# stateless-consensus/phant

Measured on NVIDIA H100. Metric: mpt_proofs_verified_per_sec, higher is better.
Workload: dtype u64

## Files before the change

phant_b200/csrc/keccak_f1600.cuh:

```cuda
#pragma once
#include <stdint.h>

namespace phant {

__constant__ uint64_t KECCAK_RC[24] = {
    0x0000000000000001ull, 0x0000000000008082ull, 0x800000000000808aull, 0x8000000080008000ull,
    0x000000000000808bull, 0x0000000080000001ull, 0x8000000080008081ull, 0x8000000000008009ull,
    0x000000000000008aull, 0x0000000000000088ull, 0x0000000080008009ull, 0x000000008000000aull,
    0x000000008000808bull, 0x800000000000008bull, 0x8000000000008089ull, 0x8000000000008003ull,
    0x8000000000008002ull, 0x8000000000000080ull, 0x000000000000800aull, 0x800000008000000aull,
    0x8000000080008081ull, 0x8000000000008080ull, 0x0000000080000001ull, 0x8000000080008008ull};

constexpr int KECCAK_RATE = 136;
constexpr int KECCAK_RATE_WORDS = 17;

template <int N>
__device__ __forceinline__ uint64_t rol64(uint64_t x)
{
    if constexpr (N == 0) return x;
    const uint32_t lo = (uint32_t)x, hi = (uint32_t)(x >> 32);
    uint32_t rlo, rhi;
    if constexpr (N == 32) {
        rlo = hi; rhi = lo;
    } else if constexpr (N < 32) {
        rlo = __funnelshift_l(hi, lo, N);
        rhi = __funnelshift_l(lo, hi, N);
    } else {
        rlo = __funnelshift_l(lo, hi, N - 32);
        rhi = __funnelshift_l(hi, lo, N - 32);
    }
    return ((uint64_t)rhi << 32) | rlo;
}

#define PHANT_RHOPI(I, J, R) b[J] = rol64<R>(a[I] ^ c[((I) % 5 + 4) % 5] ^ r1[((I) % 5 + 1) % 5]);

__device__ __forceinline__ void keccak_round(uint64_t (&a)[25], uint64_t rc)
{
    uint64_t c[5], r1[5], b[25];
#pragma unroll
    for (int x = 0; x < 5; ++x) c[x] = a[x] ^ a[x + 5] ^ a[x + 10] ^ a[x + 15] ^ a[x + 20];
#pragma unroll
    for (int x = 0; x < 5; ++x) r1[x] = rol64<1>(c[x]);
    PHANT_RHOPI(0, 0, 0)    PHANT_RHOPI(1, 10, 1)   PHANT_RHOPI(2, 20, 62)  PHANT_RHOPI(3, 5, 28)   PHANT_RHOPI(4, 15, 27)
    PHANT_RHOPI(5, 16, 36)  PHANT_RHOPI(6, 1, 44)   PHANT_RHOPI(7, 11, 6)   PHANT_RHOPI(8, 21, 55)  PHANT_RHOPI(9, 6, 20)
    PHANT_RHOPI(10, 7, 3)   PHANT_RHOPI(11, 17, 10) PHANT_RHOPI(12, 2, 43)  PHANT_RHOPI(13, 12, 25) PHANT_RHOPI(14, 22, 39)
    PHANT_RHOPI(15, 23, 41) PHANT_RHOPI(16, 8, 45)  PHANT_RHOPI(17, 18, 15) PHANT_RHOPI(18, 3, 21)  PHANT_RHOPI(19, 13, 8)
    PHANT_RHOPI(20, 14, 18) PHANT_RHOPI(21, 24, 2)  PHANT_RHOPI(22, 9, 61)  PHANT_RHOPI(23, 19, 56) PHANT_RHOPI(24, 4, 14)
#pragma unroll
    for (int y = 0; y < 25; y += 5) {
#pragma unroll
        for (int x = 0; x < 5; ++x) a[y + x] = b[y + x] ^ (~b[y + (x + 1) % 5] & b[y + (x + 2) % 5]);
    }
    a[0] ^= rc;
}

__device__ __forceinline__ void keccak_last_round_digest(uint64_t (&a)[25], uint64_t rc)
{
    uint64_t c[5], r1[5], b[5];
#pragma unroll
    for (int x = 0; x < 5; ++x) c[x] = a[x] ^ a[x + 5] ^ a[x + 10] ^ a[x + 15] ^ a[x + 20];
#pragma unroll
    for (int x = 0; x < 5; ++x) r1[x] = rol64<1>(c[x]);
    PHANT_RHOPI(0, 0, 0) PHANT_RHOPI(6, 1, 44) PHANT_RHOPI(12, 2, 43) PHANT_RHOPI(18, 3, 21) PHANT_RHOPI(24, 4, 14)
#pragma unroll
    for (int x = 0; x < 4; ++x) a[x] = b[x] ^ (~b[(x + 1) % 5] & b[(x + 2) % 5]);
    a[0] ^= rc;
}
#undef PHANT_RHOPI

template <int UNROLL = 2, bool DIGEST_ONLY = false>
__device__ __forceinline__ void keccak_f1600(uint64_t (&a)[25])
{
    constexpr int LOOPED = DIGEST_ONLY ? 24 - UNROLL : 24;
#pragma unroll 1
    for (int r = 0; r < LOOPED; r += UNROLL) {
#pragma unroll
        for (int k = 0; k < UNROLL; ++k) keccak_round(a, KECCAK_RC[r + k]);
    }
    if constexpr (DIGEST_ONLY) {
#pragma unroll
        for (int k = 0; k < UNROLL - 1; ++k) keccak_round(a, KECCAK_RC[LOOPED + k]);
        keccak_last_round_digest(a, KECCAK_RC[23]);
    }
}

struct MsgView {
    const uint64_t* w;
    uint32_t sh;
};
__device__ __forceinline__ MsgView msg_view(const void* p)
{
    const uintptr_t a = (uintptr_t)p;
    return MsgView{(const uint64_t*)(a & ~(uintptr_t)7), (uint32_t)(a & 7) * 8};
}
__device__ __forceinline__ uint64_t funnel64(uint64_t lo, uint64_t hi, uint32_t sh)
{
    return sh ? (lo >> sh) | (hi << (64 - sh)) : lo;
}

template <int UNROLL>
__device__ __forceinline__ void absorb_full(uint64_t (&st)[25], const MsgView& v, uint32_t base)
{
    uint64_t w[KECCAK_RATE_WORDS + 1];
#pragma unroll
    for (int k = 0; k < KECCAK_RATE_WORDS; ++k) w[k] = v.w[base + k];
    w[KECCAK_RATE_WORDS] = v.sh ? v.w[base + KECCAK_RATE_WORDS] : 0;
#pragma unroll
    for (int k = 0; k < KECCAK_RATE_WORDS; ++k) st[k] ^= funnel64(w[k], w[k + 1], v.sh);
    keccak_f1600<UNROLL>(st);
}

template <int UNROLL>
__device__ __forceinline__ void absorb_final(uint64_t (&st)[25], const MsgView& v, uint32_t base, uint32_t rem)
{
    const uint32_t mis = v.sh >> 3;
#pragma unroll
    for (int k = 0; k < KECCAK_RATE_WORDS; ++k) {
        const int valid = (int)rem - 8 * k;
        uint64_t word = 0;
        if (valid > 0) {
            const uint64_t lo = v.w[base + k];
            const uint64_t hi = (mis + (valid > 8 ? 8 : valid) > 8) ? v.w[base + k + 1] : 0;
            word = funnel64(lo, hi, v.sh);
            if (valid < 8) word &= (1ull << (8 * valid)) - 1;
        }
        if (valid >= 0 && valid < 8) word ^= 1ull << (8 * valid);
        st[k] ^= word;
    }
    st[KECCAK_RATE_WORDS - 1] ^= 0x8000000000000000ull;
    keccak_f1600<UNROLL, true>(st);
}

#ifndef PHANT_HOST_SMEM
__device__ __forceinline__ uint32_t lds32(uint32_t saddr)
{
    uint32_t v;
    asm volatile("ld.shared.u32 %0, [%1];" : "=r"(v) : "r"(saddr));
    return v;
}
#else
__device__ __forceinline__ uint32_t lds32(uint32_t saddr) { uint32_t v; memcpy(&v, PHANT_HOST_SMEM + saddr, 4); return v; }
#endif
template <int UNROLL, bool DIGEST_ONLY = false>
__device__ __forceinline__ void absorb_full_smem(uint64_t (&st)[25], uint32_t sa)
{
    const uint32_t a4 = sa & ~3u, sh = (sa & 3u) * 8;
    uint32_t w[2 * KECCAK_RATE_WORDS + 1];
#pragma unroll
    for (int j = 0; j < 2 * KECCAK_RATE_WORDS; ++j) w[j] = lds32(a4 + 4 * j);
    w[2 * KECCAK_RATE_WORDS] = sh ? lds32(a4 + 4 * 2 * KECCAK_RATE_WORDS) : 0;
#pragma unroll
    for (int k = 0; k < KECCAK_RATE_WORDS; ++k) {
        const uint32_t lo = __funnelshift_r(w[2 * k], w[2 * k + 1], sh);
        const uint32_t hi = __funnelshift_r(w[2 * k + 1], w[2 * k + 2], sh);
        st[k] ^= ((uint64_t)hi << 32) | lo;
    }
    keccak_f1600<UNROLL, DIGEST_ONLY>(st);
}
#ifndef PHANT_HOST_SMEM
__device__ __forceinline__ void sts32_(uint32_t saddr, uint32_t v) { asm volatile("st.shared.u32 [%0], %1;" ::"r"(saddr), "r"(v) : "memory"); }
#else
__device__ __forceinline__ void sts32_(uint32_t saddr, uint32_t v) { memcpy(PHANT_HOST_SMEM + saddr, &v, 4); }
#endif
template <int UNROLL>
__device__ __forceinline__ void absorb_final_smem_masked(uint64_t (&st)[25], uint32_t sa, uint32_t rem)
{
    const uint32_t a4 = sa & ~3u, sh = (sa & 3u) * 8;
    const uint32_t nfw = rem >> 2, tail = rem & 3u;
    const uint32_t bmask = (1u << (8 * tail)) - 1u, pad = 1u << (8 * tail);
    uint32_t prev = rem ? lds32(a4) : 0;
#pragma unroll
    for (int j = 0; j < 2 * KECCAK_RATE_WORDS; ++j) {
        uint32_t word = 0;
        if ((uint32_t)j < nfw || ((uint32_t)j == nfw && tail)) {
            const uint32_t next = lds32(a4 + 4 * (j + 1));
            word = __funnelshift_r(prev, next, sh);
            prev = next;
        }
        if ((uint32_t)j == nfw) word = (word & bmask) ^ pad;
        if (j == 2 * KECCAK_RATE_WORDS - 1) word ^= 0x80000000u;
        st[j >> 1] ^= (j & 1) ? ((uint64_t)word << 32) : (uint64_t)word;
    }
    keccak_f1600<UNROLL, true>(st);
}
template <int UNROLL>
__device__ __forceinline__ void absorb_final_smem(uint64_t (&st)[25], uint32_t sa, uint32_t rem, uint32_t room)
{
    if (room < KECCAK_RATE + 4) { absorb_final_smem_masked<UNROLL>(st, sa, rem); return; }
    const uint32_t a4 = sa & ~3u, s = sa & 3u;
    const uint32_t p0 = rem + s, p1 = KECCAK_RATE - 1 + s;
    const uint32_t q0 = p0 >> 2, b0 = p0 & 3u, q1 = p1 >> 2, b1 = p1 & 3u;
    uint32_t w0 = lds32(a4 + 4 * q0);
    w0 = (w0 & ((1u << (8 * b0)) - 1u)) | (1u << (8 * b0));
    if (q0 == q1) w0 |= 0x80u << (8 * b1);
    sts32_(a4 + 4 * q0, w0);
    for (uint32_t q = q0 + 1; q < q1; ++q) sts32_(a4 + 4 * q, 0u);
    if (q1 > q0) sts32_(a4 + 4 * q1, 0x80u << (8 * b1));
    absorb_full_smem<UNROLL, true>(st, sa);
}

template <int UNROLL = 2>
__device__ __forceinline__ void keccak256_thread(const uint8_t* p, uint64_t len, uint64_t (&digest)[4])
{
    uint64_t st[25];
#pragma unroll
    for (int i = 0; i < 25; ++i) st[i] = 0;
    const MsgView v = msg_view(p);
    uint32_t base = 0;
    while (len >= KECCAK_RATE) {
        absorb_full<UNROLL>(st, v, base);
        base += KECCAK_RATE_WORDS;
        len -= KECCAK_RATE;
    }
    absorb_final<UNROLL>(st, v, base, (uint32_t)len);
#pragma unroll
    for (int i = 0; i < 4; ++i) digest[i] = st[i];
}

}
```

phant_b200/csrc/keccak_kernels.cu:

```cuda
#include "common.cuh"
#include "keccak_f1600.cuh"
#include "node_summary.cuh"
#include "stage.cuh"

#include <stdlib.h>
#include <string.h>

namespace phant {

template <int UNROLL>
__global__ void __launch_bounds__(128)
keccak256_direct_kernel(const uint8_t* __restrict__ msgs, const uint64_t* __restrict__ off,
                        const uint32_t* __restrict__ order, uint64_t n, uint8_t* __restrict__ out,
                        uint32_t* __restrict__ summary, const uint64_t* __restrict__ len)
{
    for (uint64_t i = (uint64_t)blockIdx.x * blockDim.x + threadIdx.x; i < n; i += (uint64_t)gridDim.x * blockDim.x) {
        const uint64_t m = order ? order[i] : i;
        const uint64_t beg = off[m], end = len ? beg + len[m] : off[m + 1];
        uint64_t dg[4];
        keccak256_thread<UNROLL>(msgs + beg, end - beg, dg);
        if (summary) summary[m] = (end - beg) <= 4096 ? summarize_node(msgs + beg, (uint32_t)(end - beg)) : 0;
        uint64_t* o = reinterpret_cast<uint64_t*>(out + 32 * m);
        o[0] = dg[0]; o[1] = dg[1]; o[2] = dg[2]; o[3] = dg[3];
    }
}


template <int UNROLL, int BLOCKS, int WARPS>
__global__ void __launch_bounds__(WARPS * 32)
keccak256_staged_kernel(const uint8_t* __restrict__ msgs, const uint64_t* __restrict__ off,
                        const uint32_t* __restrict__ order, uint64_t n, uint8_t* __restrict__ out,
                        uint32_t* __restrict__ summary, const uint64_t* __restrict__ len)
{
    extern __shared__ __align__(128) uint8_t smem[];
    const uint32_t warp = threadIdx.x >> 5, lane = threadIdx.x & 31;
    const uint32_t bar = smem_u32(smem) + 8 * warp;
    constexpr int SLOT = stage_slot(BLOCKS), WINDOW = stage_window(BLOCKS);
    uint8_t* slot = smem + 128 + (warp * 32 + lane) * SLOT;
    const uint32_t slot_s = smem_u32(slot);
    if (lane == 0) mbar_init(bar, 32);
    fence_proxy_async();
    __syncthreads();
    uint32_t parity = 0;

    const uint64_t n_tiles = (n + 31) / 32;
    for (uint64_t tile = (uint64_t)blockIdx.x * WARPS + warp; tile < n_tiles; tile += (uint64_t)gridDim.x * WARPS) {
        const uint64_t idx = tile * 32 + lane;
        const bool active = idx < n;
        uint64_t m = 0, cur = 0, end = 0;
        if (active) {
            m = order ? order[idx] : idx;
            cur = off[m];
            end = len ? cur + len[m] : off[m + 1];
        }
        uint64_t st[25];
#pragma unroll
        for (int i = 0; i < 25; ++i) st[i] = 0;
        bool done = !active;
        bool first_trip = true;

        while (!__all_sync(0xffffffffu, done)) {
            const uint64_t need = done ? 0 : end - cur;
            const uint64_t a0 = cur & ~(uint64_t)15;
            uint32_t cs = 0;
            if (need) {
                const uint64_t span = ((end - a0) + 15) & ~(uint64_t)15;
                cs = span < WINDOW ? (uint32_t)span : WINDOW;
                fence_proxy_async();
                mbar_arrive_expect_tx(bar, cs);
                bulk_g2s(slot_s, msgs + a0, cs, bar);
            } else {
                mbar_arrive(bar);
            }
            mbar_wait(bar, parity);
            parity ^= 1;
            if (!done) {
                const uint32_t skew = (uint32_t)(cur - a0);
                const uint64_t in_slot = cs - skew;
                const uint64_t avail = need < in_slot ? need : in_slot;
                if (summary && first_trip)
                    summary[m] = avail == need ? summarize_node(slot + skew, (uint32_t)need) : 0;
                const uint32_t nfull = (uint32_t)(avail / KECCAK_RATE);
                uint32_t sa = slot_s + skew;
                for (uint32_t b = 0; b < nfull; ++b) {
                    absorb_full_smem<UNROLL>(st, sa);
                    sa += KECCAK_RATE;
                }
                if (avail == need) {
                    absorb_final_smem<UNROLL>(st, sa, (uint32_t)(avail - (uint64_t)nfull * KECCAK_RATE), slot_s + SLOT - sa);
                    done = true;
                } else {
                    cur += (uint64_t)nfull * KECCAK_RATE;
                }
            }
            first_trip = false;
        }
        if (active) {
            uint4* o = reinterpret_cast<uint4*>(out + 32 * m);
            o[0] = make_uint4((uint32_t)st[0], (uint32_t)(st[0] >> 32), (uint32_t)st[1], (uint32_t)(st[1] >> 32));
            o[1] = make_uint4((uint32_t)st[2], (uint32_t)(st[2] >> 32), (uint32_t)st[3], (uint32_t)(st[3] >> 32));
        }
    }
}

__device__ __forceinline__ uint64_t rolv64(uint64_t x, uint32_t n) { return n ? (x << n) | (x >> (64 - n)) : x; }

__global__ void __launch_bounds__(256)
keccak256_warp_kernel(const uint8_t* __restrict__ msgs, const uint64_t* __restrict__ off, uint64_t n,
                      uint8_t* __restrict__ out, const uint64_t* __restrict__ lens)
{
    const uint32_t lane = threadIdx.x & 31;
    const uint64_t warp_id = ((uint64_t)blockIdx.x * blockDim.x + threadIdx.x) >> 5;
    const uint64_t n_warps = ((uint64_t)gridDim.x * blockDim.x) >> 5;
    const uint32_t x = lane % 5, y = (lane % 25) / 5;
    constexpr uint32_t RHO[25] = {0, 1, 62, 28, 27, 36, 44, 6, 55, 20, 3, 10, 43, 25, 39, 41, 45, 15, 21, 8, 18, 2, 61, 56, 14};
    uint32_t rho = 0;
#pragma unroll
    for (int i = 0; i < 25; ++i) if (lane == (uint32_t)i) rho = RHO[i];
    const uint32_t pi_src = ((x + 3 * y) % 5) + 5 * x;
    const uint32_t col1 = (x + 1) % 5, col4 = (x + 4) % 5;
    const uint32_t row1 = 5 * y + (x + 1) % 5, row2 = 5 * y + (x + 2) % 5;
    const uint32_t FULL = 0xffffffffu;

    for (uint64_t m = warp_id; m < n; m += n_warps) {
        const uint64_t beg = off[m], end = lens ? beg + lens[m] : off[m + 1];
        uint64_t len = end - beg;
        const MsgView v = msg_view(msgs + beg);
        uint64_t s = 0;
        uint32_t base = 0;
        bool last = false;
        while (!last) {
            uint64_t word = 0;
            if (len >= KECCAK_RATE) {
                uint64_t lo = 0;
                if (lane <= KECCAK_RATE_WORDS && (lane < KECCAK_RATE_WORDS || v.sh)) lo = v.w[base + lane];
                const uint64_t hi = __shfl_down_sync(FULL, lo, 1);
                word = lane < KECCAK_RATE_WORDS ? funnel64(lo, hi, v.sh) : 0;
                len -= KECCAK_RATE;
                base += KECCAK_RATE_WORDS;
            } else {
                const uint32_t rem = (uint32_t)len, mis = v.sh >> 3;
                const uint32_t n_al = (mis + rem + 7) / 8;
                uint64_t lo = (rem && lane < n_al) ? v.w[base + lane] : 0;
                const uint64_t hi = __shfl_down_sync(FULL, lo, 1);
                if (lane < KECCAK_RATE_WORDS) {
                    const int valid = (int)rem - 8 * (int)lane;
                    if (valid > 0) {
                        word = funnel64(lo, hi, v.sh);
                        if (valid < 8) word &= (1ull << (8 * valid)) - 1;
                    }
                    if (valid >= 0 && valid < 8) word ^= 1ull << (8 * valid);
                    if (lane == KECCAK_RATE_WORDS - 1) word ^= 0x8000000000000000ull;
                }
                last = true;
            }
            s ^= word;
#pragma unroll 1
            for (int r = 0; r < 24; ++r) {
                uint64_t c = s;
                c ^= __shfl_sync(FULL, s, (lane + 5) % 25);
                c ^= __shfl_sync(FULL, s, (lane + 10) % 25);
                c ^= __shfl_sync(FULL, s, (lane + 15) % 25);
                c ^= __shfl_sync(FULL, s, (lane + 20) % 25);
                const uint64_t cm = __shfl_sync(FULL, c, col4), cp = __shfl_sync(FULL, c, col1);
                s ^= cm ^ rolv64(cp, 1);
                s = rolv64(s, rho);
                s = __shfl_sync(FULL, s, pi_src);
                const uint64_t b1 = __shfl_sync(FULL, s, row1), b2 = __shfl_sync(FULL, s, row2);
                s ^= ~b1 & b2;
                if (lane == 0) s ^= KECCAK_RC[r];
            }
        }
        if (lane < 4) reinterpret_cast<uint64_t*>(out + 32 * m)[lane] = s;
    }
}

constexpr int CLS_THREADS = 256, CLS_WARPS = CLS_THREADS / 32;

__device__ __forceinline__ uint32_t keccak_class_of(uint64_t len)
{
    const uint64_t nb = len / KECCAK_RATE + 1;
    return (uint32_t)(15 - (nb > 16 ? 15 : nb - 1));
}
__device__ __forceinline__ uint32_t proof_class_of(uint64_t n_nodes) { return (uint32_t)(15 - (n_nodes > 15 ? 15 : n_nodes)); }
template <bool PROOFS>
__device__ __forceinline__ uint32_t class_of(uint64_t len) { return PROOFS ? proof_class_of(len) : keccak_class_of(len); }

template <bool PROOFS>
__global__ void __launch_bounds__(CLS_THREADS)
keccak_class_kernel(const uint64_t* __restrict__ off, uint64_t n, uint64_t chunk, uint32_t* __restrict__ hist ,
                    uint32_t* __restrict__ ticket, unsigned long long* __restrict__ perms)
{
    __shared__ uint32_t h[16];
    __shared__ uint32_t cls_total[16];
    __shared__ bool last;
    if (threadIdx.x < 16) h[threadIdx.x] = 0;
    __syncthreads();
    const uint64_t lo = (uint64_t)blockIdx.x * chunk, hi = lo + chunk < n ? lo + chunk : n;
    unsigned long long local = 0;
    for (uint64_t i0 = lo; i0 < hi; i0 += CLS_THREADS) {
        const uint64_t i = i0 + threadIdx.x;
        const bool valid = i < hi;
        uint32_t c = 16;
        if (valid) {
            const uint64_t len = off[i + 1] - off[i];
            c = class_of<PROOFS>(len);
            if (!PROOFS) local += len / KECCAK_RATE + 1;
        }
        const uint32_t peers = __match_any_sync(0xffffffffu, c);
        if (valid && (threadIdx.x & 31) == (uint32_t)(__ffs(peers) - 1)) atomicAdd(&h[c], __popc(peers));
    }
    for (int o = 16; o; o >>= 1) local += __shfl_down_sync(0xffffffffu, local, o);
    if ((threadIdx.x & 31) == 0 && local) atomicAdd(perms, local);
    __syncthreads();
    if (threadIdx.x < 16) hist[16 * blockIdx.x + threadIdx.x] = h[threadIdx.x];
    __threadfence();
    __syncthreads();
    if (threadIdx.x == 0) last = atomicAdd(ticket, 1u) == gridDim.x - 1;
    __syncthreads();
    if (!last) return;
    __threadfence();
    const uint32_t nb = gridDim.x, warp = threadIdx.x >> 5, lane = threadIdx.x & 31;
    for (uint32_t c = warp; c < 16; c += CLS_WARPS) {
        uint32_t t = 0;
        for (uint32_t b = lane; b < nb; b += 32) t += __ldcg(&hist[16 * b + c]);
        for (int o = 16; o; o >>= 1) t += __shfl_down_sync(0xffffffffu, t, o);
        if (lane == 0) cls_total[c] = t;
    }
    __syncthreads();
    for (uint32_t c = warp; c < 16; c += CLS_WARPS) {
        uint32_t carry = 0;
        for (uint32_t k = 0; k < c; ++k) carry += cls_total[k];
        for (uint32_t b0 = 0; b0 < nb; b0 += 32) {
            const uint32_t b = b0 + lane;
            const uint32_t v = b < nb ? __ldcg(&hist[16 * b + c]) : 0;
            uint32_t incl = v;
            for (int o = 1; o < 32; o <<= 1) {
                const uint32_t up = __shfl_up_sync(0xffffffffu, incl, o);
                if (lane >= (uint32_t)o) incl += up;
            }
            if (b < nb) hist[16 * b + c] = carry + incl - v;
            carry += __shfl_sync(0xffffffffu, incl, 31);
// ... 154 lines not shown
```

phant_b200/csrc/verify_fused.cu:

```cuda
#include "common.cuh"
#include "stage.cuh"
#include "verify_fused.cuh"

namespace phant {

template <int UNROLL, int BLOCKS, int WARPS>
__global__ void __launch_bounds__(WARPS * 32)
verify_fused_kernel(const uint8_t* __restrict__ nodes, const uint64_t* __restrict__ node_off, const uint64_t* __restrict__ proof_first,
                    const uint32_t* __restrict__ order, uint64_t n, const uint8_t* __restrict__ keys32, const uint8_t* __restrict__ roots32,
                    uint64_t n_roots, uint8_t* __restrict__ status, uint64_t* __restrict__ val_off, uint32_t* __restrict__ val_len,
                    unsigned long long* __restrict__ perms)
{
    extern __shared__ __align__(128) uint8_t smem[];
    const uint32_t warp = threadIdx.x >> 5, lane = threadIdx.x & 31;
    const uint32_t bar = smem_u32(smem) + 8 * warp;
    constexpr int SLOT = stage_slot(BLOCKS), WINDOW = stage_window(BLOCKS);
    uint8_t* slot = smem + 128 + (warp * 32 + lane) * SLOT;
    const uint32_t slot_s = smem_u32(slot);
    if (lane == 0) mbar_init(bar, 32);
    fence_proxy_async();
    __syncthreads();
    uint32_t parity = 0;
    unsigned long long my_perms = 0;

    const uint64_t n_tiles = (n + 31) / 32;
    for (uint64_t tile = (uint64_t)blockIdx.x * WARPS + warp; tile < n_tiles; tile += (uint64_t)gridDim.x * WARPS) {
        const uint64_t idx = tile * 32 + lane;
        const bool active = idx < n;
        uint64_t p = 0;
        FusedLane L;
        L.done = true;
        if (active) {
            p = order ? order[idx] : idx;
            fused_begin(L, node_off, proof_first[p], proof_first[p + 1], keys32 + 32 * p, roots32 + (n_roots == 1 ? 0 : 32 * p));
        }
        while (!__all_sync(0xffffffffu, L.done)) {
            uint64_t a0 = 0;
            const uint32_t cs = L.done ? 0 : fused_window<WINDOW>(L, a0);
            if (cs) {
                fence_proxy_async();
                mbar_arrive_expect_tx(bar, cs);
                bulk_g2s(slot_s, nodes + a0, cs, bar);
            } else {
                mbar_arrive(bar);
            }
            mbar_wait(bar, parity);
            parity ^= 1;
            if (!L.done) fused_step<UNROLL, SLOT>(L, nodes, node_off, slot_s, slot, cs);
        }
        if (active) {
            status[p] = (uint8_t)L.status;
            if (val_off) val_off[p] = L.voff;
            if (val_len) val_len[p] = L.vlen;
            my_perms += L.perms;
        }
    }
    for (int o = 16; o; o >>= 1) my_perms += __shfl_down_sync(0xffffffffu, my_perms, o);
    if (lane == 0 && my_perms) atomicAdd(perms, my_perms);
}

cudaError_t launch_verify_fused(cudaStream_t s, int device, const uint8_t* nodes, const uint64_t* node_off, const uint64_t* proof_first,
                                const uint32_t* order, uint64_t n, const uint8_t* keys32, const uint8_t* roots32, uint64_t n_roots,
                                uint8_t* status, uint64_t* val_off, uint32_t* val_len, unsigned long long* perms)
{
    if (n == 0) return cudaSuccess;
    constexpr int BLOCKS = 4, WARPS = 12;
    constexpr int SMEM = stage_smem(BLOCKS, WARPS);
    static int ctas_cache[64] = {0};
    int& ctas_per_sm = ctas_cache[(device >= 0 && device < 64) ? device : 0];
    if (!ctas_per_sm) {
        cudaError_t e = cudaFuncSetAttribute(verify_fused_kernel<2, BLOCKS, WARPS>, cudaFuncAttributeMaxDynamicSharedMemorySize, SMEM);
        if (e != cudaSuccess) return e;
        cudaFuncSetAttribute(verify_fused_kernel<2, BLOCKS, WARPS>, cudaFuncAttributePreferredSharedMemoryCarveout, 100);
        e = cudaOccupancyMaxActiveBlocksPerMultiprocessor(&ctas_per_sm, verify_fused_kernel<2, BLOCKS, WARPS>, WARPS * 32, SMEM);
        if (e != cudaSuccess || ctas_per_sm < 1) { ctas_per_sm = 0; return e != cudaSuccess ? e : cudaErrorLaunchOutOfResources; }
    }
    const uint64_t tiles = (n + 31) / 32;
    uint64_t blocks = (tiles + WARPS - 1) / WARPS;
    const uint64_t cap = (uint64_t)keccak_num_sms(device) * ctas_per_sm;
    if (blocks > cap) blocks = cap;
    verify_fused_kernel<2, BLOCKS, WARPS><<<(unsigned)blocks, WARPS * 32, SMEM, s>>>(nodes, node_off, proof_first, order, n, keys32, roots32,
                                                                                    n_roots, status, val_off, val_len, perms);
    return cudaGetLastError();
}


}
```

phant_b200/csrc/verify_fused.cuh:

```cuda
#pragma once
#include <stdint.h>

#include "keccak_f1600.cuh"
#include "node_summary.cuh"
#include "walk_one.cuh"

namespace phant {
namespace {

struct FusedLane {
    uint64_t st[25];
    uint32_t expect[8];
    uint32_t kw[8];
    uint32_t pos;
    uint64_t i, last;
    uint64_t cur, end;
    uint64_t voff;
    uint32_t vlen;
    uint64_t perms;
    int status;
    bool done;
    bool fresh;
};

__device__ __forceinline__ uint64_t node_perms(uint64_t len) { return len / KECCAK_RATE + 1; }

__device__ __forceinline__ void fused_finish(FusedLane& L, const uint64_t* __restrict__ node_off, int status)
{
    L.status = status;
    L.done = true;
    for (uint64_t j = L.i + 1; j < L.last; ++j) L.perms += node_perms(node_off[j + 1] - node_off[j]);
}

__device__ __forceinline__ void fused_enter(FusedLane& L, const uint64_t* __restrict__ node_off)
{
    L.cur = node_off[L.i];
    L.end = node_off[L.i + 1];
#pragma unroll
    for (int k = 0; k < 25; ++k) L.st[k] = 0;
    L.fresh = true;
    L.perms += node_perms(L.end - L.cur);
    if (L.end - L.cur > 0xffffffffull) fused_finish(L, node_off, ST_REJECT);
}

__device__ __forceinline__ void fused_begin(FusedLane& L, const uint64_t* __restrict__ node_off, uint64_t first, uint64_t last,
                                            const uint8_t* __restrict__ key, const uint8_t* __restrict__ root)
{
    L.voff = 0;
    L.vlen = 0;
    L.perms = 0;
    L.pos = 0;
    L.done = false;
    L.status = ST_REJECT;
    load32_aligned(root, L.expect);
    load32_aligned(key, L.kw);
    L.i = first;
    L.last = last;
    if (first == last) {
        L.status = eq32_const(EMPTY_ROOT, L.expect) ? ST_ABSENT : ST_REJECT;
        L.done = true;
        return;
    }
    fused_enter(L, node_off);
}

template <int WINDOW>
__device__ __forceinline__ uint32_t fused_window(const FusedLane& L, uint64_t& a0)
{
    a0 = L.cur & ~(uint64_t)15;
    if (L.end == L.cur) return 0;
    const uint64_t span = ((L.end - a0) + 15) & ~(uint64_t)15;
    return span < (uint64_t)WINDOW ? (uint32_t)span : (uint32_t)WINDOW;
}

template <int UNROLL, int SLOT>
__device__ __forceinline__ void fused_step(FusedLane& L, const uint8_t* __restrict__ nodes, const uint64_t* __restrict__ node_off,
                                           uint32_t slot_s, const uint8_t* slot, uint32_t cs)
{
    const uint64_t need = L.end - L.cur;
    const uint32_t skew = (uint32_t)(L.cur & 15);
    const uint64_t in_slot = (uint64_t)cs - skew;
    const uint64_t avail = need < in_slot ? need : in_slot;
    const uint32_t nfull = (uint32_t)(avail / KECCAK_RATE);
    uint32_t sa = slot_s + skew;
    for (uint32_t b = 0; b < nfull; ++b) {
        absorb_full_smem<UNROLL>(L.st, sa);
        sa += KECCAK_RATE;
    }
    if (avail != need) {
        L.cur += (uint64_t)nfull * KECCAK_RATE;
        L.fresh = false;
        return;
    }
    absorb_final_smem<UNROLL>(L.st, sa, (uint32_t)(avail - (uint64_t)nfull * KECCAK_RATE), slot_s + SLOT - sa);
    uint32_t diff = 0;
#pragma unroll
    for (int k = 0; k < 4; ++k) diff |= ((uint32_t)L.st[k] ^ L.expect[2 * k]) | ((uint32_t)(L.st[k] >> 32) ^ L.expect[2 * k + 1]);
    if (diff) { fused_finish(L, node_off, ST_REJECT); return; }
    const bool is_last = L.i + 1 == L.last;
    const uint64_t beg = L.fresh ? L.cur : node_off[L.i];
    const uint32_t len = (uint32_t)(L.end - beg);
    const uint32_t sm = L.fresh ? summarize_node(slot + skew, len) : 0;
    int r;
    if ((sm & 3u) == 1u && L.pos < 64) {
        const uint32_t nibble = key_nibble(L.kw, L.pos);
        ++L.pos;
        const uint32_t mask = sm >> 8;
        if (!((mask >> nibble) & 1u)) { fused_finish(L, node_off, is_last ? ST_ABSENT : ST_REJECT); return; }
        const uint32_t before = __popc(mask & ((1u << nibble) - 1u));
        const uint32_t ra = slot_s + skew + ((sm >> 2) & 7u) + 33u * before + (nibble - before) + 1u;
        const uint32_t a4 = ra & ~3u, sh = (ra & 3u) * 8;
        uint32_t w[9];
#pragma unroll
        for (int k = 0; k < 9; ++k) w[k] = lds32(a4 + 4 * k);
#pragma unroll
        for (int k = 0; k < 8; ++k) L.expect[k] = __funnelshift_r(w[k], w[k + 1], sh);
        r = WALK_NEXT;
    } else {
        r = walk_node(nodes, nodes + beg, len, 0, is_last, L.kw, L.pos, L.expect, L.voff, L.vlen);
    }
    if (r != WALK_NEXT) { fused_finish(L, node_off, r); return; }
    if (is_last) { fused_finish(L, node_off, ST_REJECT); return; }
    ++L.i;
    fused_enter(L, node_off);
}

}
}
```

phant_b200/csrc/walk_one.cuh:

```cuda
#pragma once
#include <stdint.h>

namespace phant {
namespace {

enum { ST_REJECT = 0, ST_PRESENT = 1, ST_ABSENT = 2, ST_MISSING = 3 };

constexpr uint32_t BAG_EMPTY = 0xffffffffu;
struct Bag {
    const uint32_t* table;
    uint32_t mask;
};

struct Item {
    uint32_t is_list;
    uint32_t pay_off;
    uint32_t pay_len;
};

__device__ __forceinline__ uint32_t rlp_item(const uint8_t* p, uint32_t avail, Item& it)
{
    if (avail == 0) return 0;
    const uint32_t b = p[0];
    if (b < 0x80) { it.is_list = 0; it.pay_off = 0; it.pay_len = 1; return 1; }
    const uint32_t is_list = b >= 0xc0;
    const uint32_t base_short = is_list ? 0xc0 : 0x80, base_long = is_list ? 0xf7 : 0xb7;
    it.is_list = is_list;
    if (b <= base_long) {
        const uint32_t len = b - base_short;
        if (1 + len > avail) return 0;
        if (!is_list && len == 1 && p[1] < 0x80) return 0;
        it.pay_off = 1; it.pay_len = len;
        return 1 + len;
    }
    const uint32_t n = b - base_long;
    if (n > 4 || 1 + n > avail) return 0;
    if (p[1] == 0) return 0;
    uint64_t len = 0;
    for (uint32_t i = 0; i < n; ++i) len = (len << 8) | p[1 + i];
    if (len <= 55) return 0;
    if (1 + n + len > avail) return 0;
    it.pay_off = 1 + n; it.pay_len = (uint32_t)len;
    return (uint32_t)(1 + n + len);
}

__device__ __forceinline__ void load32_aligned(const uint8_t* a, uint32_t (&e)[8])
{
    const uint4 lo = __ldg(reinterpret_cast<const uint4*>(a)), hi = __ldg(reinterpret_cast<const uint4*>(a) + 1);
    e[0] = lo.x; e[1] = lo.y; e[2] = lo.z; e[3] = lo.w;
    e[4] = hi.x; e[5] = hi.y; e[6] = hi.z; e[7] = hi.w;
}
__device__ __forceinline__ bool eq32_aligned(const uint8_t* a, const uint32_t (&e)[8])
{
    uint32_t d[8];
    load32_aligned(a, d);
    uint32_t diff = 0;
#pragma unroll
    for (int i = 0; i < 8; ++i) diff |= d[i] ^ e[i];
    return diff == 0;
}
__device__ __forceinline__ void load32(const uint8_t* a, uint32_t (&e)[8])
{
    const uintptr_t p = (uintptr_t)a;
    const uint4* q = reinterpret_cast<const uint4*>(p & ~(uintptr_t)15);
    const uint4 q0 = __ldg(q), q1 = __ldg(q + 1), q2 = __ldg(q + 2);
    const uint32_t v[12] = {q0.x, q0.y, q0.z, q0.w, q1.x, q1.y, q1.z, q1.w, q2.x, q2.y, q2.z, q2.w};
    const uint32_t w0 = (uint32_t)(p & 15) >> 2, sh = (uint32_t)(p & 3) * 8;
    uint32_t u[9];
#pragma unroll
    for (int i = 0; i < 9; ++i) {
        const uint32_t a01 = (w0 & 1) ? v[i + 1] : v[i];
        const uint32_t a23 = (w0 & 1) ? v[i + 3 < 12 ? i + 3 : 11] : v[i + 2 < 12 ? i + 2 : 11];
        u[i] = (w0 & 2) ? a23 : a01;
    }
#pragma unroll
    for (int i = 0; i < 8; ++i) e[i] = __funnelshift_r(u[i], u[i + 1], sh);
}
__device__ __forceinline__ bool eq32_const(const uint8_t* a, const uint32_t (&e)[8])
{
    uint32_t diff = 0;
#pragma unroll
    for (int i = 0; i < 8; ++i) {
        const uint32_t w = (uint32_t)a[4 * i] | ((uint32_t)a[4 * i + 1] << 8) | ((uint32_t)a[4 * i + 2] << 16) | ((uint32_t)a[4 * i + 3] << 24);
        diff |= w ^ e[i];
    }
    return diff == 0;
}

__constant__ uint8_t EMPTY_ROOT[32] = {0x56, 0xe8, 0x1f, 0x17, 0x1b, 0xcc, 0x55, 0xa6, 0xff, 0x83, 0x45,
                                       0xe6, 0x92, 0xc0, 0xf8, 0x6e, 0x5b, 0x48, 0xe0, 0x1b, 0x99, 0x6c,
                                       0xad, 0xc0, 0x01, 0x62, 0x2f, 0xb5, 0xe3, 0x63, 0xb4, 0x21};

__device__ __forceinline__ uint32_t bag_slot(const uint32_t (&e)[8], uint32_t mask)
{
    uint64_t h = ((uint64_t)e[1] << 32) | e[0];
    h ^= h >> 29; h *= 0xBF58476D1CE4E5B9ull; h ^= h >> 32;
    return (uint32_t)h & mask;
}
__device__ uint32_t bag_find(const Bag& bag, const uint8_t* __restrict__ digests, const uint32_t (&expect)[8])
{
    uint32_t s = bag_slot(expect, bag.mask);
    for (;;) {
        const uint32_t idx = bag.table[s];
        if (idx == BAG_EMPTY) return BAG_EMPTY;
        if (eq32_aligned(digests + 32ull * idx, expect)) return idx;
        s = (s + 1) & bag.mask;
    }
}

__device__ __forceinline__ uint32_t key_nibble(const uint32_t (&kw)[8], uint32_t q)
{
    const uint32_t wi = q >> 3;
    const uint32_t a01 = (wi & 1) ? kw[1] : kw[0], a23 = (wi & 1) ? kw[3] : kw[2], a45 = (wi & 1) ? kw[5] : kw[4], a67 = (wi & 1) ? kw[7] : kw[6];
    const uint32_t lo4 = (wi & 2) ? a23 : a01, hi4 = (wi & 2) ? a67 : a45;
    const uint32_t w = (wi & 4) ? hi4 : lo4;
    const uint32_t byte = (w >> (8 * ((q >> 1) & 3))) & 0xffu;
    return (q & 1) ? (byte & 15u) : (byte >> 4);
}

constexpr int WALK_NEXT = -1;

__device__ __forceinline__ int walk_node(const uint8_t* nodes, const uint8_t* cur, uint32_t cur_len, uint32_t sm, bool is_last,
                                         const uint32_t (&kw)[8], uint32_t& pos, uint32_t (&expect)[8], uint64_t& voff, uint32_t& vlen)
{
    if ((sm & 3u) == 1u && pos < 64) {
        const uint32_t nibble = key_nibble(kw, pos);
        ++pos;
        const uint32_t mask = sm >> 8;
        if (!((mask >> nibble) & 1u)) return is_last ? ST_ABSENT : ST_REJECT;
        const uint32_t before = __popc(mask & ((1u << nibble) - 1u));
        load32(cur + ((sm >> 2) & 7u) + 33u * before + (nibble - before) + 1u, expect);
        return WALK_NEXT;
    }
    for (;;) {
        Item top;
        const uint32_t tot = rlp_item(cur, cur_len, top);
        if (tot == 0 || !top.is_list || tot != cur_len) return ST_REJECT;
        const uint8_t* pay = cur + top.pay_off;
        const uint32_t pl = top.pay_len;

        const uint32_t want = pos < 64 ? key_nibble(kw, pos) : 16u;
        Item it0{}, it1{}, itw{}, it16{};
        uint32_t off0 = 0, off1 = 0, offw = 0, off16 = 0;
        uint32_t cnt = 0, o = 0;
        while (o < pl) {
            if (cnt == 17) return ST_REJECT;
            Item it;
            const uint32_t t = rlp_item(pay + o, pl - o, it);
            if (t == 0) return ST_REJECT;
            if (cnt == 0) { it0 = it; off0 = o; }
            if (cnt == 1) { it1 = it; off1 = o; }
            if (cnt == want) { itw = it; offw = o; }
            if (cnt == 16) { it16 = it; off16 = o; }
            o += t;
            ++cnt;
        }
        if (cnt != 17 && cnt != 2) return ST_REJECT;

        Item child;
        uint32_t child_off;
        if (cnt == 17) {
            if (pos == 64) {
                if (it16.is_list || !is_last) return ST_REJECT;
                if (it16.pay_len == 0) return ST_ABSENT;
                voff = (uint64_t)(pay + off16 + it16.pay_off - nodes);
                vlen = it16.pay_len;
                return ST_PRESENT;
            }
            child = itw; child_off = offw;
            ++pos;
        } else {
            if (it0.is_list || it0.pay_len == 0) return ST_REJECT;
            const uint8_t* hp = pay + off0 + it0.pay_off;
            const uint32_t flag = hp[0] >> 4;
            if (flag > 3) return ST_REJECT;
            if (!(flag & 1) && (hp[0] & 15)) return ST_REJECT;
            const uint32_t plen = 2 * (it0.pay_len - 1) + (flag & 1);
            if (plen > 64) return ST_REJECT;
            bool match = 64 - pos >= plen;
            if ((flag & 2) && pos + plen != 64) match = false;
            else if (match && (flag & 2) && plen >= 2 && (uint64_t)(hp + it0.pay_len - nodes) >= 48) {
                uint32_t tail[8];
                load32(hp + it0.pay_len - 32, tail);
                const uint32_t nb = plen >> 1;
                uint32_t diff = 0;
#pragma unroll
                for (int w = 0; w < 8; ++w) {
                    const int first = 32 - (int)nb - 4 * w;
                    const uint32_t m = first <= 0 ? 0xffffffffu : (first >= 4 ? 0u : 0xffffffffu << (8 * first));
                    diff |= (tail[w] ^ kw[w]) & m;
                }
                if ((flag & 1) && (hp[0] & 15u) != key_nibble(kw, pos)) diff = 1;
                match = diff == 0;
            } else if (match) {
                for (uint32_t j = 0; j < plen; ++j) {
                    const uint32_t q = j + 2 - (flag & 1);
                    const uint32_t pn = (q & 1) ? (hp[q >> 1] & 15u) : (hp[q >> 1] >> 4);
                    if (pn != key_nibble(kw, pos + j)) { match = false; break; }
                }
            }
            if (flag & 2) {
                if (it1.is_list || !is_last) return ST_REJECT;
                if (match && pos + plen == 64) {
                    voff = (uint64_t)(pay + off1 + it1.pay_off - nodes);
                    vlen = it1.pay_len;
                    return ST_PRESENT;
                }
                return ST_ABSENT;
            }
            if (plen == 0) return ST_REJECT;
            if (!match) return is_last ? ST_ABSENT : ST_REJECT;
            pos += plen;
            child = it1; child_off = off1;
        }
        if (child.is_list) {
            const uint32_t tot_child = child.pay_off + child.pay_len;
            if (tot_child >= 32) return ST_REJECT;
            cur = pay + child_off;
            cur_len = tot_child;
            continue;
        }
        if (child.pay_len == 0) {
            if (cnt == 2) return ST_REJECT;
            return is_last ? ST_ABSENT : ST_REJECT;
        }
        if (child.pay_len != 32) return ST_REJECT;
        load32(pay + child_off + child.pay_off, expect);
        return WALK_NEXT;
    }
}

template <bool BAG>
__device__ int walk_one(const uint8_t* __restrict__ nodes, const uint64_t* __restrict__ node_off,
                        const uint64_t* __restrict__ node_index, const Bag bag, uint64_t first,
                        uint64_t last, const uint8_t* __restrict__ key, const uint8_t* __restrict__ root,
                        const uint8_t* __restrict__ digests, const uint32_t* __restrict__ summary, uint64_t& voff, uint32_t& vlen)
{
    voff = 0; vlen = 0;
    uint32_t expect[8];
    load32_aligned(root, expect);
    uint32_t kw[8];
    load32_aligned(key, kw);
    if (BAG) {
        first = 0;
        last = 1;
        if (eq32_const(EMPTY_ROOT, expect)) return ST_ABSENT;
    } else if (first == last) return eq32_const(EMPTY_ROOT, expect) ? ST_ABSENT : ST_REJECT;

    uint32_t pos = 0;
    uint64_t i = first;
    for (;;) {
        uint64_t ni;
        if (BAG) {
            const uint32_t f = bag_find(bag, digests, expect);
            if (f == BAG_EMPTY) return ST_MISSING;
            ni = f;
            i = last - 1;
        } else {
            if (i == last) return ST_REJECT;
            ni = node_index ? node_index[i] : i;
        }
        const uint64_t o = node_off[ni];
        const uint64_t l = node_off[ni + 1] - o;
        if (l > 0xffffffffull) return ST_REJECT;
        if (!BAG && !eq32_aligned(digests + 32 * ni, expect)) return ST_REJECT;
        const uint32_t sm = summary ? summary[ni] : 0;
        ++i;
        const int r = walk_node(nodes, nodes + o, (uint32_t)l, sm, i == last, kw, pos, expect, voff, vlen);
        if (r != WALK_NEXT) return r;
    }
}

}
}
```

Measured before the change: 119.2 million.

## Walk staged nodes from shared memory and initialize sponge state on first absorb

Makes walk_node generic over a byte source so the fused verifier can parse RLP, compare extension keys and read child hashes straight from the node bytes already staged in the lane's shared-memory slot, not from global memory. This covers every node that fits in the slot in one trip, extending the earlier shared-memory path that only handled branch summaries. The sponge state is no longer zeroed up front; the first absorb writes the block and clears the capacity words, and fused_enter reuses the previous end offset instead of reloading node_off. This adds template and control complexity and relies on the staged window covering the whole node.

```diff
diff --git a/phant_b200/csrc/keccak_f1600.cuh b/phant_b200/csrc/keccak_f1600.cuh
--- a/phant_b200/csrc/keccak_f1600.cuh
+++ b/phant_b200/csrc/keccak_f1600.cuh
@@ -141,20 +141,34 @@
 #else
 __device__ __forceinline__ uint32_t lds32(uint32_t saddr) { uint32_t v; memcpy(&v, PHANT_HOST_SMEM + saddr, 4); return v; }
 #endif
+__device__ __forceinline__ void absorb_words(uint64_t (&st)[25], const uint64_t (&blk)[KECCAK_RATE_WORDS], bool fresh)
+{
+    if (fresh) {
+#pragma unroll
+        for (int k = 0; k < KECCAK_RATE_WORDS; ++k) st[k] = blk[k];
+#pragma unroll
+        for (int k = KECCAK_RATE_WORDS; k < 25; ++k) st[k] = 0;
+    } else {
+#pragma unroll
+        for (int k = 0; k < KECCAK_RATE_WORDS; ++k) st[k] ^= blk[k];
+    }
+}
 template <int UNROLL, bool DIGEST_ONLY = false>
-__device__ __forceinline__ void absorb_full_smem(uint64_t (&st)[25], uint32_t sa)
+__device__ __forceinline__ void absorb_full_smem(uint64_t (&st)[25], uint32_t sa, bool fresh = false)
 {
     const uint32_t a4 = sa & ~3u, sh = (sa & 3u) * 8;
     uint32_t w[2 * KECCAK_RATE_WORDS + 1];
 #pragma unroll
     for (int j = 0; j < 2 * KECCAK_RATE_WORDS; ++j) w[j] = lds32(a4 + 4 * j);
     w[2 * KECCAK_RATE_WORDS] = sh ? lds32(a4 + 4 * 2 * KECCAK_RATE_WORDS) : 0;
+    uint64_t blk[KECCAK_RATE_WORDS];
 #pragma unroll
     for (int k = 0; k < KECCAK_RATE_WORDS; ++k) {
         const uint32_t lo = __funnelshift_r(w[2 * k], w[2 * k + 1], sh);
         const uint32_t hi = __funnelshift_r(w[2 * k + 1], w[2 * k + 2], sh);
-        st[k] ^= ((uint64_t)hi << 32) | lo;
-    }
+        blk[k] = ((uint64_t)hi << 32) | lo;
+    }
+    absorb_words(st, blk, fresh);
     keccak_f1600<UNROLL, DIGEST_ONLY>(st);
 }
 #ifndef PHANT_HOST_SMEM
@@ -163,12 +177,13 @@
 __device__ __forceinline__ void sts32_(uint32_t saddr, uint32_t v) { memcpy(PHANT_HOST_SMEM + saddr, &v, 4); }
 #endif
 template <int UNROLL>
-__device__ __forceinline__ void absorb_final_smem_masked(uint64_t (&st)[25], uint32_t sa, uint32_t rem)
+__device__ __forceinline__ void absorb_final_smem_masked(uint64_t (&st)[25], uint32_t sa, uint32_t rem, bool fresh)
 {
     const uint32_t a4 = sa & ~3u, sh = (sa & 3u) * 8;
     const uint32_t nfw = rem >> 2, tail = rem & 3u;
     const uint32_t bmask = (1u << (8 * tail)) - 1u, pad = 1u << (8 * tail);
     uint32_t prev = rem ? lds32(a4) : 0;
+    uint64_t blk[KECCAK_RATE_WORDS];
 #pragma unroll
     for (int j = 0; j < 2 * KECCAK_RATE_WORDS; ++j) {
         uint32_t word = 0;
@@ -179,14 +194,16 @@
         }
         if ((uint32_t)j == nfw) word = (word & bmask) ^ pad;
         if (j == 2 * KECCAK_RATE_WORDS - 1) word ^= 0x80000000u;
-        st[j >> 1] ^= (j & 1) ? ((uint64_t)word << 32) : (uint64_t)word;
-    }
+        if (j & 1) blk[j >> 1] |= (uint64_t)word << 32;
+        else blk[j >> 1] = word;
+    }
+    absorb_words(st, blk, fresh);
     keccak_f1600<UNROLL, true>(st);
 }
 template <int UNROLL>
-__device__ __forceinline__ void absorb_final_smem(uint64_t (&st)[25], uint32_t sa, uint32_t rem, uint32_t room)
-{
-    if (room < KECCAK_RATE + 4) { absorb_final_smem_masked<UNROLL>(st, sa, rem); return; }
+__device__ __forceinline__ void absorb_final_smem(uint64_t (&st)[25], uint32_t sa, uint32_t rem, uint32_t room, bool fresh = false)
+{
+    if (room < KECCAK_RATE + 4) { absorb_final_smem_masked<UNROLL>(st, sa, rem, fresh); return; }
     const uint32_t a4 = sa & ~3u, s = sa & 3u;
     const uint32_t p0 = rem + s, p1 = KECCAK_RATE - 1 + s;
     const uint32_t q0 = p0 >> 2, b0 = p0 & 3u, q1 = p1 >> 2, b1 = p1 & 3u;
@@ -196,7 +213,7 @@
     sts32_(a4 + 4 * q0, w0);
     for (uint32_t q = q0 + 1; q < q1; ++q) sts32_(a4 + 4 * q, 0u);
     if (q1 > q0) sts32_(a4 + 4 * q1, 0x80u << (8 * b1));
-    absorb_full_smem<UNROLL, true>(st, sa);
+    absorb_full_smem<UNROLL, true>(st, sa, fresh);
 }
 
 template <int UNROLL = 2>
diff --git a/phant_b200/csrc/keccak_kernels.cu b/phant_b200/csrc/keccak_kernels.cu
--- a/phant_b200/csrc/keccak_kernels.cu
+++ b/phant_b200/csrc/keccak_kernels.cu
@@ -54,8 +54,6 @@
             end = len ? cur + len[m] : off[m + 1];
         }
         uint64_t st[25];
-#pragma unroll
-        for (int i = 0; i < 25; ++i) st[i] = 0;
         bool done = !active;
         bool first_trip = true;
 
@@ -83,11 +81,12 @@
                 const uint32_t nfull = (uint32_t)(avail / KECCAK_RATE);
                 uint32_t sa = slot_s + skew;
                 for (uint32_t b = 0; b < nfull; ++b) {
-                    absorb_full_smem<UNROLL>(st, sa);
+                    absorb_full_smem<UNROLL>(st, sa, first_trip && b == 0);
                     sa += KECCAK_RATE;
                 }
                 if (avail == need) {
-                    absorb_final_smem<UNROLL>(st, sa, (uint32_t)(avail - (uint64_t)nfull * KECCAK_RATE), slot_s + SLOT - sa);
+                    absorb_final_smem<UNROLL>(st, sa, (uint32_t)(avail - (uint64_t)nfull * KECCAK_RATE), slot_s + SLOT - sa,
+                                              first_trip && nfull == 0);
                     done = true;
                 } else {
                     cur += (uint64_t)nfull * KECCAK_RATE;
diff --git a/phant_b200/csrc/verify_fused.cu b/phant_b200/csrc/verify_fused.cu
--- a/phant_b200/csrc/verify_fused.cu
+++ b/phant_b200/csrc/verify_fused.cu
@@ -15,6 +15,7 @@
     const uint32_t warp = threadIdx.x >> 5, lane = threadIdx.x & 31;
     const uint32_t bar = smem_u32(smem) + 8 * warp;
     constexpr int SLOT = stage_slot(BLOCKS), WINDOW = stage_window(BLOCKS);
+    static_assert(WINDOW + 4 <= SLOT, "the slot walk must stay inside the lane's slot");
     uint8_t* slot = smem + 128 + (warp * 32 + lane) * SLOT;
     const uint32_t slot_s = smem_u32(slot);
     if (lane == 0) mbar_init(bar, 32);
diff --git a/phant_b200/csrc/verify_fused.cuh b/phant_b200/csrc/verify_fused.cuh
--- a/phant_b200/csrc/verify_fused.cuh
+++ b/phant_b200/csrc/verify_fused.cuh
@@ -34,10 +34,8 @@
 
 __device__ __forceinline__ void fused_enter(FusedLane& L, const uint64_t* __restrict__ node_off)
 {
-    L.cur = node_off[L.i];
+    L.cur = L.end;
     L.end = node_off[L.i + 1];
-#pragma unroll
-    for (int k = 0; k < 25; ++k) L.st[k] = 0;
     L.fresh = true;
     L.perms += node_perms(L.end - L.cur);
     if (L.end - L.cur > 0xffffffffull) fused_finish(L, node_off, ST_REJECT);
@@ -61,6 +59,7 @@
         L.done = true;
         return;
     }
+    L.end = node_off[first];
     fused_enter(L, node_off);
 }
 
@@ -84,7 +83,7 @@
     const uint32_t nfull = (uint32_t)(avail / KECCAK_RATE);
     uint32_t sa = slot_s + skew;
     for (uint32_t b = 0; b < nfull; ++b) {
-        absorb_full_smem<UNROLL>(L.st, sa);
+        absorb_full_smem<UNROLL>(L.st, sa, L.fresh && b == 0);
         sa += KECCAK_RATE;
     }
     if (avail != need) {
@@ -92,32 +91,20 @@
         L.fresh = false;
         return;
     }
-    absorb_final_smem<UNROLL>(L.st, sa, (uint32_t)(avail - (uint64_t)nfull * KECCAK_RATE), slot_s + SLOT - sa);
+    absorb_final_smem<UNROLL>(L.st, sa, (uint32_t)(avail - (uint64_t)nfull * KECCAK_RATE), slot_s + SLOT - sa, L.fresh && nfull == 0);
     uint32_t diff = 0;
 #pragma unroll
     for (int k = 0; k < 4; ++k) diff |= ((uint32_t)L.st[k] ^ L.expect[2 * k]) | ((uint32_t)(L.st[k] >> 32) ^ L.expect[2 * k + 1]);
     if (diff) { fused_finish(L, node_off, ST_REJECT); return; }
     const bool is_last = L.i + 1 == L.last;
-    const uint64_t beg = L.fresh ? L.cur : node_off[L.i];
-    const uint32_t len = (uint32_t)(L.end - beg);
-    const uint32_t sm = L.fresh ? summarize_node(slot + skew, len) : 0;
     int r;
-    if ((sm & 3u) == 1u && L.pos < 64) {
-        const uint32_t nibble = key_nibble(L.kw, L.pos);
-        ++L.pos;
-        const uint32_t mask = sm >> 8;
-        if (!((mask >> nibble) & 1u)) { fused_finish(L, node_off, is_last ? ST_ABSENT : ST_REJECT); return; }
-        const uint32_t before = __popc(mask & ((1u << nibble) - 1u));
-        const uint32_t ra = slot_s + skew + ((sm >> 2) & 7u) + 33u * before + (nibble - before) + 1u;
-        const uint32_t a4 = ra & ~3u, sh = (ra & 3u) * 8;
-        uint32_t w[9];
-#pragma unroll
-        for (int k = 0; k < 9; ++k) w[k] = lds32(a4 + 4 * k);
-#pragma unroll
-        for (int k = 0; k < 8; ++k) L.expect[k] = __funnelshift_r(w[k], w[k + 1], sh);
-        r = WALK_NEXT;
+    if (L.fresh) {
+        const uint8_t* node = slot + skew;
+        const uint32_t len = (uint32_t)need;
+        r = walk_node(SlotBytes{node, slot_s + skew, L.cur, skew}, node, len, summarize_node(node, len), is_last, L.kw, L.pos, L.expect, L.voff, L.vlen);
     } else {
-        r = walk_node(nodes, nodes + beg, len, 0, is_last, L.kw, L.pos, L.expect, L.voff, L.vlen);
+        const uint64_t beg = node_off[L.i];
+        r = walk_node(GlobalBytes{nodes}, nodes + beg, (uint32_t)(L.end - beg), 0, is_last, L.kw, L.pos, L.expect, L.voff, L.vlen);
     }
     if (r != WALK_NEXT) { fused_finish(L, node_off, r); return; }
     if (is_last) { fused_finish(L, node_off, ST_REJECT); return; }
diff --git a/phant_b200/csrc/walk_one.cuh b/phant_b200/csrc/walk_one.cuh
--- a/phant_b200/csrc/walk_one.cuh
+++ b/phant_b200/csrc/walk_one.cuh
@@ -1,5 +1,6 @@
 #pragma once
 #include <stdint.h>
+#include <string.h>
 
 namespace phant {
 namespace {
@@ -18,10 +19,11 @@
     uint32_t pay_len;
 };
 
-__device__ __forceinline__ uint32_t rlp_item(const uint8_t* p, uint32_t avail, Item& it)
+template <class Src>
+__device__ __forceinline__ uint32_t rlp_item_at(const Src& src, const uint8_t* p, uint32_t avail, Item& it)
 {
     if (avail == 0) return 0;
-    const uint32_t b = p[0];
+    const uint32_t b = src.u8(p);
     if (b < 0x80) { it.is_list = 0; it.pay_off = 0; it.pay_len = 1; return 1; }
     const uint32_t is_list = b >= 0xc0;
     const uint32_t base_short = is_list ? 0xc0 : 0x80, base_long = is_list ? 0xf7 : 0xb7;
@@ -29,15 +31,15 @@
     if (b <= base_long) {
         const uint32_t len = b - base_short;
         if (1 + len > avail) return 0;
-        if (!is_list && len == 1 && p[1] < 0x80) return 0;
+        if (!is_list && len == 1 && src.u8(p + 1) < 0x80) return 0;
         it.pay_off = 1; it.pay_len = len;
         return 1 + len;
     }
     const uint32_t n = b - base_long;
     if (n > 4 || 1 + n > avail) return 0;
-    if (p[1] == 0) return 0;
+    if (src.u8(p + 1) == 0) return 0;
     uint64_t len = 0;
-    for (uint32_t i = 0; i < n; ++i) len = (len << 8) | p[1 + i];
+    for (uint32_t i = 0; i < n; ++i) len = (len << 8) | src.u8(p + 1 + i);
     if (len <= 55) return 0;
     if (1 + n + len > avail) return 0;
     it.pay_off = 1 + n; it.pay_len = (uint32_t)len;
@@ -87,6 +89,58 @@
     return diff == 0;
 }
 
+struct GlobalBytes {
+    const uint8_t* nodes;
+    __device__ __forceinline__ uint32_t u8(const uint8_t* p) const { return *p; }
+    __device__ __forceinline__ void load32(const uint8_t* p, uint32_t (&e)[8]) const { phant::load32(p, e); }
+    __device__ __forceinline__ uint64_t lead(const uint8_t* p) const { return (uint64_t)(p - nodes); }
+    __device__ __forceinline__ uint64_t off(const uint8_t* p) const { return (uint64_t)(p - nodes); }
+};
+__device__ __forceinline__ uint32_t rlp_item(const uint8_t* p, uint32_t avail, Item& it) { return rlp_item_at(GlobalBytes{p}, p, avail, it); }
+struct SlotBytes {
+    const uint8_t* node;
+    uint32_t node_s;
+    uint64_t at;
+    uint32_t skew;
+    __device__ __forceinline__ uint32_t sa(const uint8_t* p) const { return node_s + (uint32_t)(p - node); }
+#ifdef __CUDA_ARCH__
+    __device__ __forceinline__ static uint32_t lds(uint32_t a)
+    {
+        uint32_t v;
+        asm volatile("ld.shared.u32 %0, [%1];" : "=r"(v) : "r"(a));
+        return v;
+    }
+    __device__ __forceinline__ uint32_t u8(const uint8_t* p) const
+    {
+        uint32_t v;
+        asm volatile("ld.shared.u8 %0, [%1];" : "=r"(v) : "r"(sa(p)));
+        return v;
+    }
+    __device__ __forceinline__ void load32(const uint8_t* p, uint32_t (&e)[8]) const
+    {
+        const uint32_t a = sa(p), a4 = a & ~3u, sh = (a & 3u) * 8;
+        uint32_t w[9];
+#pragma unroll
+        for (int k = 0; k < 9; ++k) w[k] = lds(a4 + 4 * k);
+#pragma unroll
+        for (int k = 0; k < 8; ++k) e[k] = __funnelshift_r(w[k], w[k + 1], sh);
+    }
+#else
+    __device__ __forceinline__ uint32_t u8(const uint8_t* p) const { return *p; }
+    __device__ __forceinline__ void load32(const uint8_t* p, uint32_t (&e)[8]) const
+    {
+        const uint8_t* a4 = (const uint8_t*)((uintptr_t)p & ~(uintptr_t)3);
+        const uint32_t sh = (uint32_t)((uintptr_t)p & 3) * 8;
+        uint32_t w[9];
+        memcpy(w, a4, sizeof w);
+#pragma unroll
+        for (int k = 0; k < 8; ++k) e[k] = __funnelshift_r(w[k], w[k + 1], sh);
+    }
+#endif
+    __device__ __forceinline__ uint64_t lead(const uint8_t* p) const { return skew + (uint64_t)(p - node); }
+    __device__ __forceinline__ uint64_t off(const uint8_t* p) const { return at + (uint64_t)(p - node); }
+};
+
 __constant__ uint8_t EMPTY_ROOT[32] = {0x56, 0xe8, 0x1f, 0x17, 0x1b, 0xcc, 0x55, 0xa6, 0xff, 0x83, 0x45,
                                        0xe6, 0x92, 0xc0, 0xf8, 0x6e, 0x5b, 0x48, 0xe0, 0x1b, 0x99, 0x6c,
                                        0xad, 0xc0, 0x01, 0x62, 0x2f, 0xb5, 0xe3, 0x63, 0xb4, 0x21};
@@ -120,7 +174,8 @@
 
 constexpr int WALK_NEXT = -1;
 
-__device__ __forceinline__ int walk_node(const uint8_t* nodes, const uint8_t* cur, uint32_t cur_len, uint32_t sm, bool is_last,
+template <class Src>
+__device__ __forceinline__ int walk_node(const Src& src, const uint8_t* cur, uint32_t cur_len, uint32_t sm, bool is_last,
                                          const uint32_t (&kw)[8], uint32_t& pos, uint32_t (&expect)[8], uint64_t& voff, uint32_t& vlen)
 {
     if ((sm & 3u) == 1u && pos < 64) {
@@ -129,12 +184,12 @@
         const uint32_t mask = sm >> 8;
         if (!((mask >> nibble) & 1u)) return is_last ? ST_ABSENT : ST_REJECT;
         const uint32_t before = __popc(mask & ((1u << nibble) - 1u));
-        load32(cur + ((sm >> 2) & 7u) + 33u * before + (nibble - before) + 1u, expect);
+        src.load32(cur + ((sm >> 2) & 7u) + 33u * before + (nibble - before) + 1u, expect);
         return WALK_NEXT;
     }
     for (;;) {
         Item top;
-        const uint32_t tot = rlp_item(cur, cur_len, top);
+        const uint32_t tot = rlp_item_at(src, cur, cur_len, top);
         if (tot == 0 || !top.is_list || tot != cur_len) return ST_REJECT;
         const uint8_t* pay = cur + top.pay_off;
         const uint32_t pl = top.pay_len;
@@ -146,7 +201,7 @@
         while (o < pl) {
             if (cnt == 17) return ST_REJECT;
             Item it;
-            const uint32_t t = rlp_item(pay + o, pl - o, it);
+            const uint32_t t = rlp_item_at(src, pay + o, pl - o, it);
             if (t == 0) return ST_REJECT;
             if (cnt == 0) { it0 = it; off0 = o; }
             if (cnt == 1) { it1 = it; off1 = o; }
@@ -163,7 +218,7 @@
             if (pos == 64) {
                 if (it16.is_list || !is_last) return ST_REJECT;
                 if (it16.pay_len == 0) return ST_ABSENT;
-                voff = (uint64_t)(pay + off16 + it16.pay_off - nodes);
+                voff = src.off(pay + off16 + it16.pay_off);
                 vlen = it16.pay_len;
                 return ST_PRESENT;
             }
@@ -172,16 +227,17 @@
         } else {
             if (it0.is_list || it0.pay_len == 0) return ST_REJECT;
             const uint8_t* hp = pay + off0 + it0.pay_off;
-            const uint32_t flag = hp[0] >> 4;
+            const uint32_t h0 = src.u8(hp);
+            const uint32_t flag = h0 >> 4;
             if (flag > 3) return ST_REJECT;
-            if (!(flag & 1) && (hp[0] & 15)) return ST_REJECT;
+            if (!(flag & 1) && (h0 & 15)) return ST_REJECT;
             const uint32_t plen = 2 * (it0.pay_len - 1) + (flag & 1);
             if (plen > 64) return ST_REJECT;
             bool match = 64 - pos >= plen;
             if ((flag & 2) && pos + plen != 64) match = false;
-            else if (match && (flag & 2) && plen >= 2 && (uint64_t)(hp + it0.pay_len - nodes) >= 48) {
+            else if (match && (flag & 2) && plen >= 2 && src.lead(hp + it0.pay_len) >= 32) {
                 uint32_t tail[8];
-                load32(hp + it0.pay_len - 32, tail);
+                src.load32(hp + it0.pay_len - 32, tail);
                 const uint32_t nb = plen >> 1;
                 uint32_t diff = 0;
 #pragma unroll
@@ -190,19 +246,20 @@
                     const uint32_t m = first <= 0 ? 0xffffffffu : (first >= 4 ? 0u : 0xffffffffu << (8 * first));
                     diff |= (tail[w] ^ kw[w]) & m;
                 }
-                if ((flag & 1) && (hp[0] & 15u) != key_nibble(kw, pos)) diff = 1;
+                if ((flag & 1) && (h0 & 15u) != key_nibble(kw, pos)) diff = 1;
                 match = diff == 0;
             } else if (match) {
                 for (uint32_t j = 0; j < plen; ++j) {
                     const uint32_t q = j + 2 - (flag & 1);
-                    const uint32_t pn = (q & 1) ? (hp[q >> 1] & 15u) : (hp[q >> 1] >> 4);
+                    const uint32_t hb = src.u8(hp + (q >> 1));
+                    const uint32_t pn = (q & 1) ? (hb & 15u) : (hb >> 4);
                     if (pn != key_nibble(kw, pos + j)) { match = false; break; }
                 }
             }
             if (flag & 2) {
                 if (it1.is_list || !is_last) return ST_REJECT;
                 if (match && pos + plen == 64) {
-                    voff = (uint64_t)(pay + off1 + it1.pay_off - nodes);
+                    voff = src.off(pay + off1 + it1.pay_off);
                     vlen = it1.pay_len;
                     return ST_PRESENT;
                 }
@@ -225,7 +282,7 @@
             return is_last ? ST_ABSENT : ST_REJECT;
         }
         if (child.pay_len != 32) return ST_REJECT;
-        load32(pay + child_off + child.pay_off, expect);
+        src.load32(pay + child_off + child.pay_off, expect);
         return WALK_NEXT;
     }
 }
@@ -266,7 +323,7 @@
         if (!BAG && !eq32_aligned(digests + 32 * ni, expect)) return ST_REJECT;
         const uint32_t sm = summary ? summary[ni] : 0;
         ++i;
-        const int r = walk_node(nodes, nodes + o, (uint32_t)l, sm, i == last, kw, pos, expect, voff, vlen);
+        const int r = walk_node(GlobalBytes{nodes}, nodes + o, (uint32_t)l, sm, i == last, kw, pos, expect, voff, vlen);
         if (r != WALK_NEXT) return r;
     }
 }
```

Result: no change. 118.9 million (median of 6 runs) (-0.3%).
